# wgurecky/CORRLA_RS

Hardware: AMD Instinct MI355X
Metric: RSVD GFLOP/s on 16k x 16k f32 rank-128 (higher is better)
Workload: dtype f32

## Files before the change

### corrla_rs_amd/csrc/hip_backend.hpp

```cpp
#pragma once
#include <hip/hip_runtime.h>
#include <rccl/rccl.h>

#include <cmath>
#include <cstdio>
#include <cstdlib>
#include <cstring>
#include <limits>
#include <random>
#include <string>
#include <type_traits>
#include <vector>

#include "core_svd_plan.hpp"
#include "driver.hpp"
#include "hip_kernels.hpp"
#include "tsqr_kernels.hpp"
#include "jacobi_mc_kernels.hpp"
#include "ata_kernels.hpp"
#include "tall_kernels.hpp"
#include "mixed_kernels.hpp"
#include "grad_kernels.hpp"
#include "knn2_kernels.hpp"
#include "grad_wide_kernels.hpp"
// ... 541 lines not shown
    }
  }
  template <class T>
  void copy_values_out(const T* src_dev, int64_t n, T* dst, bool dst_is_host) {
    CORRLA_HIP(hipMemcpyAsync(dst, src_dev, sizeof(T) * n, dst_is_host ? hipMemcpyDeviceToHost : hipMemcpyDeviceToDevice,
                              stream));
    if (dst_is_host) sync();
  }
  template <class T>
  bool device_chol_fits(int64_t l) const {
    return l <= 4096 && k::chol_inv_fits((int)l, sizeof(T)) && !no_device_chol_;
  }
  template <class T>
  bool device_chol_blocked_fits(int64_t l) const {
    const int64_t n1 = round_up((l + 1) / 2, (int64_t)4);
    return l > 8 && l <= 4096 && k::chol_inv_fits((int)n1, sizeof(T)) && !no_device_chol_;
  }
  template <class T>
  void copy_block(const Skinny<T>& src, int64_t r0, int64_t c0, int64_t rows, int64_t cols, Skinny<T>& dst, int64_t dr0,
                  int64_t dc0) {
    if (rows <= 0 || cols <= 0) return;
    CORRLA_HIP(hipMemcpy2DAsync(dst.p + dc0 * dst.ld + dr0, (size_t)dst.ld * sizeof(T), src.p + c0 * src.ld + r0,
                                (size_t)src.ld * sizeof(T), (size_t)rows * sizeof(T), (size_t)cols, hipMemcpyDeviceToDevice,
                                stream));
  }
  template <class T>
  void chol_inv(const Skinny<T>& g, int64_t r, T piv_rel, Skinny<T>& m_out, void* st_dev, int slot) {
    hipLaunchKernelGGL((k::chol_inv_kernel<T>), dim3(1), dim3(k::chol_inv_threads((int)r)),
                       k::chol_inv_lds_bytes((int)r, sizeof(T)), stream, (const T*)g.p, g.ld, (int)r, piv_rel, m_out.p,
                       m_out.ld, (k::CholStatus*)st_dev + slot);
    CORRLA_HIP(hipGetLastError());
  }
  void set_run_if(const int* p) { run_if_ = p; }
  int robust_passes() const { return robust_passes_; }
  void set_robust_passes(int n) { robust_passes_ = n; }
  bool svd_more_sweeps() {
    if (jmc_extra_sweeps_ >= 24) return false;
    jmc_extra_sweeps_ += 8;
    jmc_sweeps_hint_ = 0;
    return true;
  }
  bool svd_force_v() {
    if (jmc_force_v_) return false;
    jmc_force_v_ = true;
    return true;
  }
  void svd_sweeps_used(int n) { jmc_sweeps_hint_ = std::max(jmc_sweeps_hint_ - 1, n); }
  int* alloc_flags(int n) { return (int*)alloc_zeroed(sizeof(int) * (size_t)std::max(n, 1)); }
  void* alloc_zeroed_bytes(size_t bytes) { return alloc_zeroed(bytes); }
  void read_bytes(const void* dev_p, size_t bytes, void* host) {
    CORRLA_HIP(hipMemcpyAsync(host, dev_p, bytes, hipMemcpyDeviceToHost, stream));
    sync();
  }
  template <class T>
  void poison_entry(Skinny<T>& s, int64_t i, int64_t j, int kind) {
    hipLaunchKernelGGL((k::poison_entry_kernel<T>), dim3(1), dim3(1), 0, stream, s.p + j * s.ld + i, kind);
    CORRLA_HIP(hipGetLastError());
  }
  struct ArenaMark {
    std::vector<size_t> used, zused;
  };
  ArenaMark arena_mark() const {
    ArenaMark mk;
    for (const auto& c : chunks_) mk.used.push_back(c.used);
    for (const auto& c : zchunks_) mk.zused.push_back(c.used);
    return mk;
  }
  void arena_rewind(const ArenaMark& mk) {
    sp_scratch_ = nullptr;
    sp_scratch_bytes_ = 0;
    for (size_t i = 0; i < chunks_.size(); ++i) chunks_[i].used = i < mk.used.size() ? mk.used[i] : 0;
    for (size_t i = 0; i < zchunks_.size(); ++i) {
      Chunk& c = zchunks_[i];
      const size_t keep = i < mk.zused.size() ? mk.zused[i] : 0;
      if (c.used > keep) CORRLA_HIP(hipMemsetAsync((char*)c.p + keep, 0, c.used - keep, stream));
      c.zeroed = std::max(c.zeroed, c.used);
      c.used = keep;
    }
  }
  int sharded_handshake(int local_status) {
    if (comm_size <= 1 && !(comm && env_int("CORRLA_FORCE_ALLREDUCE", 0))) return local_status;
    if (!comm) throw Error(ST_ECOMM, "communicator not initialised");
    double h[8] = {(double)local_status, (double)robust_passes_, (double)jmc_extra_sweeps_, (double)jmc_sweeps_hint_,
                   jmc_force_v_ ? 1.0 : 0.0, 0.0, 0.0, 0.0};
    double* d = (double*)alloc_bytes(sizeof(h));
    CORRLA_HIP(hipMemcpyAsync(d, h, sizeof(h), hipMemcpyHostToDevice, stream));
    CORRLA_NCCL(ncclAllReduce(d, d, 8, ncclDouble, ncclMax, comm, stream));
    ++n_collectives;
    collective_bytes += sizeof(h);
    CORRLA_HIP(hipMemcpyAsync(h, d, sizeof(h), hipMemcpyDeviceToHost, stream));
    sync();
    robust_passes_ = (int)h[1];
    jmc_extra_sweeps_ = (int)h[2];
    jmc_sweeps_hint_ = (int)h[3];
    jmc_force_v_ = h[4] != 0.0;
    return (int)h[0];
  }
  void read_flags(const int* dev_p, int n, int* host) {
    CORRLA_HIP(hipMemcpyAsync(host, dev_p, sizeof(int) * (size_t)n, hipMemcpyDeviceToHost, stream));
    sync();
  }
  template <class T>
  bool device_qr_robust_fits(int64_t l) const {
    return robust_qr_ && (device_chol_fits<T>(l) || device_chol_blocked_fits<T>(l));
  }
  bool qr_inplace_fits(int64_t l) const { return col_blocking(l).nblk == 1; }
  template <class T>
  void* alloc_inspect() { return alloc_zeroed(sizeof(k::GramInspect<T>)); }
  template <class T>
  const void* inspect_shift_ptr(const void* insp) const { return &((const k::GramInspect<T>*)insp)->shift; }
  template <class T>
  void gram_inspect(Skinny<T>& g, int64_t l, float shift_rel, int shift_mode, void* insp) {
    hipLaunchKernelGGL((k::gram_inspect_kernel<T>), dim3(1), dim3(1024), 0, stream, g.p, g.ld, (int)l, shift_rel, shift_mode,
                       (k::GramInspect<T>*)insp, run_if_);
    CORRLA_HIP(hipGetLastError());
  }
  template <class T>
  void combine_need(int* need, const void* insp, const int* na, const int* nb) {
    hipLaunchKernelGGL((k::combine_need_kernel<T>), dim3(1), dim3(1), 0, stream, need, (const k::GramInspect<T>*)insp, na, nb,
                       run_if_);
    CORRLA_HIP(hipGetLastError());
  }
  template <class T>
  void chol_inv_robust(const Skinny<T>& g, int64_t r, T piv_rel, float shift_rel, int shift_mode, float null_excess,
                       Skinny<T>& m_out, void* st_dev, int slot, int* need_next, int* null_mask,
                       const void* abs_shift = nullptr, float need_ratio = 0.f) {
    k::CholRobust rb{shift_rel, shift_mode, null_excess, need_next, null_mask, run_if_, need_ratio, abs_shift};
    hipLaunchKernelGGL((k::chol_inv_kernel<T>), dim3(1), dim3(k::chol_inv_threads((int)r)),
                       k::chol_inv_lds_bytes((int)r, sizeof(T)), stream, (const T*)g.p, g.ld, (int)r, piv_rel, m_out.p,
                       m_out.ld, (k::CholStatus*)st_dev + slot, rb);
    CORRLA_HIP(hipGetLastError());
  }
  template <class T>
  void apply_inplace(Skinny<T>& y, int64_t l, const Skinny<T>& m) {
    Skinny<T> out = y.view_cols(l);
    Skinny<T> mv = m.view_cols(l);
    mv.rows = l;
    launch_gemm<T>(true, as_rowmajor_transposed(y, l), mv, out, (const T*)nullptr);
  }
  template <class T>
  void refill_null(Skinny<T>& y, int64_t l, const int* null_mask, uint64_t seed) {
    const int bx = (int)std::min<int64_t>(64, (y.rows + 255) / 256);
    hipLaunchKernelGGL((k::refill_null_kernel<T>), dim3((unsigned)std::max(bx, 1), (unsigned)l), dim3(256), 0, stream, y.p, y.ld,
                       y.rows, (int)l, null_mask, seed, run_if_);
    CORRLA_HIP(hipGetLastError());
  }

  void read_chol_status(const void* st_dev, int n, int* fail, float* min_ratio, float* dev_i) {
    static_assert(sizeof(k::CholStatus) == 32, "driver.hpp assumes 32-byte status records");
    static_assert(k::kNeedNonFinite == kFlagNonFinite && k::kNeedNullCols == kFlagNullCols, "need_next bits: kernels vs driver");
    std::vector<k::CholStatus> h((size_t)std::max(n, 1));
    CORRLA_HIP(hipMemcpyAsync(h.data(), st_dev, sizeof(k::CholStatus) * n, hipMemcpyDeviceToHost, stream));
    sync();
    for (int i = 0; i < n; ++i) {
      fail[i] = h[i].fail;
      min_ratio[i] = h[i].min_ratio;
      dev_i[i] = h[i].dev_i;
      if (env_int("CORRLA_DEBUG", 0) >= 2)
        std::fprintf(stderr, "[corrla] chol_inv[%d]: fail %d min_ratio %.3g dev_i %.3g clk %lld wall %lld (%.0f MHz)\n", i,
                     h[i].fail, h[i].min_ratio, h[i].dev_i, h[i].clk, h[i].wall,
                     h[i].wall > 0 ? 100.0 * (double)h[i].clk / (double)h[i].wall : 0.0);
    }
  }

  template <class T>
  void inv_sqrt_series(Skinny<T>& g, int64_t r, Skinny<T>& m_out) {
    Skinny<T> e2 = alloc_skinny<T>(r, r), e3 = alloc_skinny<T>(r, r);
    if (e2.ld != g.ld || m_out.ld != g.ld) throw Error(ST_EINVAL, "internal: series operands must share a leading dimension");
    dim3 grid((unsigned)((r + 63) / 64), (unsigned)r);
    hipLaunchKernelGGL((k::series_prep_kernel<T>), grid, dim3(64), 0, stream, g.p, g.ld, (int)r);
    Big<T> eb;
    eb.p = g.p;
    eb.rows = r;
    eb.cols = r;
    eb.ld = g.ld;
    eb.cols_readable = g.ld;
    Skinny<T> gv = g.view_cols(r);
    gv.rows = r;
    gemm_nn(eb, gv, e2, (const T*)nullptr);
    gemm_nn(eb, e2, e3, (const T*)nullptr);
    memset_zero(m_out.p, (size_t)m_out.ld * m_out.cols_alloc * sizeof(T));
    hipLaunchKernelGGL((k::series_combine_kernel<T>), grid, dim3(64), 0, stream, (const T*)g.p, (const T*)e2.p,
                       (const T*)e3.p, g.ld, (int)r, m_out.p, m_out.ld);
    CORRLA_HIP(hipGetLastError());
  }

  bool hh_wy_ = env_int("CORRLA_HH_WY", 1) != 0;
  template <class T>
  size_t hh_panel_lds(int rows, int l) const {
    return hh_wy_ ? k::hh_wy_lds_bytes(rows, l, sizeof(T)) : k::hh_lds_bytes(rows, l, sizeof(T));
  }
  template <class T>
  bool householder_fits(int64_t l) const {
    return l >= 1 && l <= 4096 && hh_panel_lds<T>((int)(2 * l), (int)l) <= (size_t)160 * 1024 && 2 * l <= 64 * k::kHhMaxRowsPerLane;
  }
  template <class T>
  struct HhState {
    int64_t m = 0;
    int l = 0, nleaf = 0, levels = 0, max_rows = 0;
    std::vector<int> n_at;
    std::vector<T*> rbuf, cbuf, taub, vbuf, tbuf;
    T* r_root() const { return rbuf[levels]; }
  };
  template <class T>
  HhState<T> householder_up(Skinny<T>& y, Skinny<T>& tmp) {
    HhState<T> h;
    const int64_t m = y.rows;
    const int l = (int)y.cols;
    if (m < l) throw Error(ST_EINVAL, "householder_thin_q: fewer rows than columns");
    if (!householder_fits<T>(l)) throw Error(ST_EINVAL, "householder_thin_q: panel does not fit in LDS");
    const int64_t br = 2 * (int64_t)l;
    const int64_t nleaf64 = m <= br ? 1 : (m + br - 1) / br;
    if (nleaf64 > 0x3fffffff) throw Error(ST_EINVAL, "householder_thin_q: too many panels");
    h.m = m;
    h.l = l;
    h.nleaf = (int)nleaf64;
    h.max_rows = (int)std::min<int64_t>(m, br);
    const size_t lds = hh_panel_lds<T>(h.max_rows, l);
    h.n_at = {h.nleaf};
    while (h.n_at.back() > 1) h.n_at.push_back((h.n_at.back() + 1) / 2);
    h.levels = (int)h.n_at.size() - 1;
    const size_t ll = (size_t)l * l;
    h.rbuf.resize(h.levels + 1);
    h.cbuf.resize(h.levels + 1);
    h.taub.resize(h.levels + 1);
    h.vbuf.assign(h.levels + 1, nullptr);
    h.tbuf.assign(h.levels + 1, nullptr);
    const size_t tsz = (size_t)k::hh_wy_panels(l) * k::kWyNb * k::kWyNb;
    for (int k_ = 0; k_ <= h.levels; ++k_) {
      if (hh_wy_) h.tbuf[k_] = (T*)alloc_bytes(tsz * h.n_at[k_] * sizeof(T));
      h.rbuf[k_] = (T*)alloc_bytes(ll * h.n_at[k_] * sizeof(T));
      h.cbuf[k_] = (T*)alloc_bytes(ll * h.n_at[k_] * sizeof(T));
      h.taub[k_] = (T*)alloc_bytes((size_t)l * h.n_at[k_] * sizeof(T));
      if (k_ >= 1) h.vbuf[k_] = (T*)alloc_bytes(2 * ll * h.n_at[k_] * sizeof(T));
    }
    auto leaf = hh_wy_ ? k::hh_leaf_factor_kernel<T, true> : k::hh_leaf_factor_kernel<T, false>;
    auto tree = hh_wy_ ? k::hh_tree_factor_kernel<T, true> : k::hh_tree_factor_kernel<T, false>;
    hipLaunchKernelGGL(leaf, dim3((unsigned)h.nleaf), dim3(k::kHhThreads), lds, stream, (const T*)y.p, y.ld, m, l, h.nleaf, tmp.p,
                       tmp.ld, h.taub[0], h.rbuf[0], h.tbuf[0]);
    const size_t lds_tree = hh_panel_lds<T>(2 * l, l);
    for (int k_ = 1; k_ <= h.levels; ++k_)
      hipLaunchKernelGGL(tree, dim3((unsigned)h.n_at[k_]), dim3(k::kHhThreads), lds_tree, stream, (const T*)h.rbuf[k_ - 1],
                         h.n_at[k_ - 1], l, h.vbuf[k_], h.taub[k_], h.rbuf[k_], h.tbuf[k_]);
    CORRLA_HIP(hipGetLastError());
    return h;
  }
  template <class T>
  void householder_down(HhState<T>& h, Skinny<T>& y, Skinny<T>& tmp, const T* root_coef = nullptr) {
    const int l = h.l;
    const size_t lds = k::hh_lds_bytes(h.max_rows, l, sizeof(T));
    const size_t lds_tree = k::hh_lds_bytes(2 * l, l, sizeof(T));
    auto tree = hh_wy_ ? k::hh_tree_apply_kernel<T, true> : k::hh_tree_apply_kernel<T, false>;
    auto leaf = hh_wy_ ? k::hh_leaf_apply_kernel<T, true> : k::hh_leaf_apply_kernel<T, false>;
    for (int k_ = h.levels; k_ >= 1; --k_)
      hipLaunchKernelGGL(tree, dim3((unsigned)h.n_at[k_]), dim3(k::kHhThreads), lds_tree, stream,
                         (const T*)(k_ == h.levels ? root_coef : h.cbuf[k_]), (const T*)h.vbuf[k_], (const T*)h.taub[k_],
                         h.n_at[k_ - 1], l, h.cbuf[k_ - 1], (const T*)h.tbuf[k_]);
    hipLaunchKernelGGL(leaf, dim3((unsigned)h.nleaf), dim3(k::kHhThreads), lds, stream,
                       (const T*)(h.levels == 0 ? root_coef : h.cbuf[0]), (const T*)tmp.p, tmp.ld, (const T*)h.taub[0], h.m, l,
                       h.nleaf, y.p, y.ld, (const T*)h.tbuf[0]);
    CORRLA_HIP(hipGetLastError());
  }
  template <class T>
  void householder_thin_q(Skinny<T>& y, Skinny<T>& tmp) {
    HhState<T> h = householder_up(y, tmp);
    householder_down(h, y, tmp);
  }
  template <class T>
  int householder_max_width() const {
    int w = 1;
    while (householder_fits<T>(w + 1)) ++w;
    return w;
  }
  int rank() const { return comm_rank; }

  template <class T>
  int jmc_lanes(int64_t) const {
    return 16;
  }
  template <class T>
  bool jmc_geometry(int64_t l, int* nc_out, int* np_out, int* b_out) const {
    return corrla::jmc_geometry(l, (int)sizeof(T), jmc_lanes<T>(l), jmc_max_b_, env_int("CORRLA_JMC_LOCAL", 1),
                                env_int("CORRLA_JMC_NP", 0), nc_out, np_out, b_out);
  }
  template <class T, int NC>
  void jmc_launch_step(int lanes, int np, int b, T* w, T* v, int nblocks, int step, int sweep, T tol, T tol_early, T floor2, k::JmcCtl* ctl) {
    const size_t lds = k::jmc_lds_bytes(NC, b, sizeof(T), lanes);
    const unsigned threads = (unsigned)((b * lanes + 63) / 64 * 64);
    hipLaunchKernelGGL((k::jmc_step_kernel<T, NC, 16>), dim3((unsigned)np), dim3(threads), lds, stream, w, v, b, nblocks, step,
                       sweep, step == 0 ? 1 : 0, tol, tol_early, floor2, ctl, jmc_local_);
  }
  template <class T>
  void small_svd_mc(const Skinny<T>& c, int64_t l, int64_t k, Skinny<T>& m1, Skinny<T>& m2, T* s_dev, void* conv_status) {
    int nc = 0, np = 0, b = 0;
    if (!jmc_geometry<T>(l, &nc, &np, &b)) throw Error(ST_EINVAL, "internal: core too large for the multi-workgroup Jacobi");
    jmc_local_ = env_int("CORRLA_JMC_LOCAL", 1);
    const int lanes = jmc_lanes<T>(l);
    const int rp = k::jmc_pitch(nc, (int)sizeof(T), lanes), nblocks = 2 * np, ncols_pad = nblocks * b;
    T* wj = (T*)alloc_bytes((size_t)rp * ncols_pad * sizeof(T));
    T* vj = (T*)alloc_bytes((size_t)rp * ncols_pad * sizeof(T));
    k::JmcCtl* ctl = (k::JmcCtl*)alloc_bytes(sizeof(k::JmcCtl));
    k::CholStatus* st = conv_status ? (k::CholStatus*)conv_status : (k::CholStatus*)alloc_bytes(sizeof(k::CholStatus));
    const int force_v = (conv_status == nullptr || jmc_force_v_ || env_int("CORRLA_JMC_FORCE_V", 0)) ? 1 : 0;
    hipLaunchKernelGGL((k::jmc_init_kernel<T>), dim3(1), dim3(1024), 0, stream, (const T*)c.p, c.ld, (int)l, wj, vj, rp,
                       ncols_pad, force_v, ctl);
    const double eps = (double)std::numeric_limits<T>::epsilon();
    const T tol = (T)(std::sqrt((double)l) * eps);
    const T tol_early = env_int("CORRLA_JACOBI_STRICT", 0) ? tol : (T)std::sqrt(eps);
    const T floor2 = (T)((double)l * eps * eps);
    auto enqueue_sweeps = [&](int s0, int s1) {
      for (int sw = s0; sw < s1; ++sw)
        for (int step = 0; step < nblocks - 1; ++step) switch (nc) {
            case 1: jmc_launch_step<T, 1>(lanes, np, b, wj, vj, nblocks, step, sw, tol, tol_early, floor2, ctl); break;
            case 2: jmc_launch_step<T, 2>(lanes, np, b, wj, vj, nblocks, step, sw, tol, tol_early, floor2, ctl); break;
            case 3: jmc_launch_step<T, 3>(lanes, np, b, wj, vj, nblocks, step, sw, tol, tol_early, floor2, ctl); break;
            case 4: jmc_launch_step<T, 4>(lanes, np, b, wj, vj, nblocks, step, sw, tol, tol_early, floor2, ctl); break;
            case 5: jmc_launch_step<T, 5>(lanes, np, b, wj, vj, nblocks, step, sw, tol, tol_early, floor2, ctl); break;
            case 6: jmc_launch_step<T, 6>(lanes, np, b, wj, vj, nblocks, step, sw, tol, tol_early, floor2, ctl); break;
            case 7: jmc_launch_step<T, 7>(lanes, np, b, wj, vj, nblocks, step, sw, tol, tol_early, floor2, ctl); break;
            case 8: jmc_launch_step<T, 8>(lanes, np, b, wj, vj, nblocks, step, sw, tol, tol_early, floor2, ctl); break;
            default: jmc_launch_step<T, 9>(lanes, np, b, wj, vj, nblocks, step, sw, tol, tol_early, floor2, ctl); break;
          }
      CORRLA_HIP(hipGetLastError());
    };
    const size_t lds_fin = (size_t)(l + 2) * sizeof(T) + (size_t)(l + 2) * sizeof(int) + 64;
    auto finish = [&](int nsw) {
      hipLaunchKernelGGL((k::jmc_finish_kernel<T>), dim3(1), dim3(1024), lds_fin, stream, (const T*)wj, (const T*)vj, rp, (int)l,
                         nsw, (const k::JmcCtl*)ctl, m1.p, m1.ld, m2.p, m2.ld, s_dev, (int)k, st);
      const unsigned groups = (unsigned)(l * k);
      hipLaunchKernelGGL((k::jmc_other_factor_kernel<T>), dim3((groups * 16 + 255) / 256), dim3(256), 0, stream, (const T*)c.p,
                         c.ld, (int)l, (int)k, (const T*)m2.p, m2.ld, (const T*)s_dev, (const k::JmcCtl*)ctl, m1.p, m1.ld);
      CORRLA_HIP(hipGetLastError());
    };
    if (conv_status) {
      const int nsw_default = std::max(1, env_int("CORRLA_JMC_SWEEPS", sizeof(T) == 4 ? 10 : 13));
      const int nsw = std::min(k::kJmcMaxSweeps, (jmc_sweeps_hint_ > 0 ? std::min(nsw_default, jmc_sweeps_hint_ + 2) : nsw_default) + jmc_extra_sweeps_);
      enqueue_sweeps(0, nsw);
      finish(nsw);
      if (env_int("CORRLA_DEBUG", 0)) {
        k::JmcCtl hd;
        CORRLA_HIP(hipMemcpyAsync(&hd, ctl, sizeof(hd), hipMemcpyDeviceToHost, stream));
        sync();
        int used = 0;
        while (used < nsw && hd.rot[used] && hd.big[used]) ++used;
        std::fprintf(stderr, "[corrla] jacobi_svd (multi-workgroup, %d sweeps enqueued, %s) l=%d np=%d b=%d nc=%d sweeps run=%d rounds(wg0)=%llu "
                             "cycles/round=%.0f ns/round=%.0f (%.0f MHz)\n", nsw, hd.with_v ? "V accumulated" : "W only", (int)l, np, b, nc, std::min(used + 1, nsw),
                     hd.rounds, hd.rounds ? (double)hd.clk / hd.rounds : 0.0, hd.rounds ? 10.0 * hd.wall / hd.rounds : 0.0,
                     hd.wall ? 100.0 * hd.clk / hd.wall : 0.0);
        if (hd.steps)
          std::fprintf(stderr, "[corrla]   per step (wg0, us): load %.2f norms %.2f rounds %.2f store %.2f total %.2f over %llu steps\n",
                       0.01 * hd.t_load / hd.steps, 0.01 * hd.t_norm / hd.steps, 0.01 * hd.wall / hd.steps,
                       0.01 * hd.t_store / hd.steps, 0.01 * hd.t_total / hd.steps, hd.steps);
        if (hd.steps > 1)
          std::fprintf(stderr, "[corrla]   span first-start..last-end over all workgroups: %.2f us per step\n",
                       0.01 * hd.t_span / (hd.steps - 1));
      }
      return;
    }
    int done = 0;
    k::JmcCtl h;
    while (done < k::kJmcMaxSweeps) {
      const int s1 = std::min(k::kJmcMaxSweeps, done + 8);
      enqueue_sweeps(done, s1);
      CORRLA_HIP(hipMemcpyAsync(&h, ctl, sizeof(h), hipMemcpyDeviceToHost, stream));
      sync();
      bool conv = false;
      for (int s_ = 0; s_ < s1; ++s_) conv = conv || !(h.rot[s_] && h.big[s_]);
      done = s1;
      if (conv || h.bad) break;
    }
    if (h.bad) throw Error(ST_ENUMERIC, "non-finite core matrix in small SVD");
    finish(done);
    if (env_int("CORRLA_DEBUG", 0)) {
      int used = 0;
      while (used < done && h.rot[used] && h.big[used]) ++used;
      std::fprintf(stderr, "[corrla] jacobi_svd (multi-workgroup) l=%d np=%d b=%d sweeps=%d\n", (int)l, np, b, used + 1);
    }
  }

  template <class T>
  void small_svd(const Skinny<T>& c, int64_t l, int64_t k, Skinny<T>& m1, Skinny<T>& m2, T* s_dev, void* conv_status) {
    if (conv_status) memset_zero(conv_status, sizeof(k::CholStatus));
    CoreSvdKnobs kn;
    kn.mode = std::getenv("CORRLA_SVD");
    kn.host_svd = env_int("CORRLA_HOST_SVD", 0) != 0;
    kn.jmc_min_l = jmc_min_l_;
    kn.jmc_max_b = jmc_max_b_;
    kn.jmc_local = env_int("CORRLA_JMC_LOCAL", 1);
    kn.jmc_np = env_int("CORRLA_JMC_NP", 0);
    const CoreSvdPlan plan = core_svd_plan((int)sizeof(T), l, kn);
    switch (plan.family) {
      case CoreSvd::kMultiWg:
        small_svd_mc(c, l, k, m1, m2, s_dev, conv_status);
        return;
      case CoreSvd::kHost:
        small_svd_host(*this, c, l, k, m1, m2, s_dev);
        return;
      case CoreSvd::kBlock:
        core_finite_check<T>(c, l, conv_status);
        small_svd_block(c, l, k, m1, m2, s_dev);
        return;
      case CoreSvd::kRing:
        core_finite_check<T>(c, l, conv_status);
        small_svd_ring(c, l, k, m1, m2, s_dev, plan.ring_e);
        return;
    }
  }
  template <class T>
  void core_finite_check(const Skinny<T>& c, int64_t l, void* conv_status) {
    int* bad = conv_status ? nullptr : alloc_flags(1);
    hipLaunchKernelGGL((k::core_finite_check_kernel<T>), dim3(1), dim3(1024), 0, stream, (const T*)c.p, c.ld, (int)l,
                       (k::CholStatus*)conv_status, bad);
    CORRLA_HIP(hipGetLastError());
    if (bad) {
      int h = 0;
      read_flags(bad, 1, &h);
      if (h) throw Error(ST_ENUMERIC, "non-finite core matrix in small SVD");
    }
  }

  template <class T>
  void small_svd_block(const Skinny<T>& c, int64_t l, int64_t k, Skinny<T>& m1, Skinny<T>& m2, T* s_dev) {
    const int nb = (int)(2 * ((l + 15) / 16));
    const int cols_pad = nb * 8;
    const int rows_pad = (int)round_up(l, 16);
    const int64_t ld = rows_pad;
    T* wj = (T*)alloc_bytes((size_t)ld * cols_pad * sizeof(T));
    T* vj = (T*)alloc_bytes((size_t)ld * cols_pad * sizeof(T));
    k::JacobiCtl* ctl = (k::JacobiCtl*)alloc_bytes(sizeof(k::JacobiCtl));
    hipLaunchKernelGGL((k::jacobi_init_kernel<T>), dim3(64), dim3(256), 0, stream, (const T*)c.p, c.ld, (int)l, wj, ld, vj,
                       ld, cols_pad, rows_pad, ctl);
    const double eps = (double)std::numeric_limits<T>::epsilon();
    const float tol_early = (float)std::sqrt(eps);
    const size_t lds = (size_t)(2 * 16 * (rows_pad + 1) + 7 * 16 * 17 + 32) * sizeof(T) + 16 * sizeof(int) + 64;
    const int max_sweeps = env_int("CORRLA_JACOBI_SWEEPS", 12), inner = env_int("CORRLA_JACOBI_INNER", 1);
    for (int sw = 0; sw < max_sweeps; ++sw) {
      for (int round = 0; round < nb - 1; ++round)
        hipLaunchKernelGGL((k::jacobi_block_round_kernel<T>), dim3(nb / 2), dim3(256), lds, stream, wj, ld, vj, ld, rows_pad,
                           nb, round, inner, ctl);
      hipLaunchKernelGGL(k::jacobi_sweep_end_kernel, dim3(1), dim3(1), 0, stream, ctl, tol_early);
    }
    const size_t lds_fin = (size_t)(l + 2) * sizeof(T) + (size_t)(l + 2) * sizeof(int) + 64;
    hipLaunchKernelGGL((k::jacobi_finish_kernel<T>), dim3(1), dim3(1024), lds_fin, stream, (const T*)wj, ld, (const T*)vj,
                       ld, (int)l, m1.p, m1.ld, m2.p, m2.ld, s_dev, (int)k);
    CORRLA_HIP(hipGetLastError());
    if (env_int("CORRLA_DEBUG", 0)) {
      k::JacobiCtl h;
      CORRLA_HIP(hipMemcpyAsync(&h, ctl, sizeof(h), hipMemcpyDeviceToHost, stream));
      sync();
      std::fprintf(stderr, "[corrla] block jacobi l=%d nb=%d sweeps=%u done=%u\n", (int)l, nb, h.sweeps, h.done);
    }
  }

  template <class T>
  void small_svd_ring(const Skinny<T>& c, int64_t l, int64_t k, Skinny<T>& m1, Skinny<T>& m2, T* s_dev, int e) {
    int* info = (int*)alloc_bytes(sizeof(int) * 4);
    const double eps = (double)std::numeric_limits<T>::epsilon();
    const T tol = (T)(std::sqrt((double)l) * eps);
    const T tol_early = env_int("CORRLA_JACOBI_STRICT", 0) ? tol : (T)std::sqrt(eps);
    const size_t ring_lds = k::jacobi_ring_w_lds_bytes((int)l, 8 * e, sizeof(T));
    const int np = (int)((l + 1) / 2);
    const dim3 block((unsigned)(np * 8));
    const int max_sw = env_int("CORRLA_JACOBI_SWEEPS", 40);
    const int n2 = 2 * np;
    k::RotEntry<T>* rot = (k::RotEntry<T>*)alloc_bytes((size_t)max_sw * n2 * k::kRingProcPad * sizeof(k::RotEntry<T>));
    int* rank_g = (int*)alloc_bytes(sizeof(int) * (size_t)n2);
#define CORRLA_RING_W(EE)                                                                                             \
  hipLaunchKernelGGL((k::jacobi_ring_w_kernel<T, EE, 8>), dim3(1), block, ring_lds, stream, (const T*)c.p, c.ld, (int)l, \
                     m2.p, m2.ld, s_dev, (int)k, tol, tol_early, max_sw, rot, rank_g, info)
    constexpr int kBigE = sizeof(T) == 4 ? 20 : 18;
    switch (e) {
      case 8: CORRLA_RING_W(8); break;
      case 12: CORRLA_RING_W(12); break;
      case 16: CORRLA_RING_W(16); break;
      default: CORRLA_RING_W(kBigE); break;
    }
#undef CORRLA_RING_W
    CORRLA_HIP(hipGetLastError());
    hipLaunchKernelGGL((k::jacobi_replay_v_kernel<T>), dim3((unsigned)((l + 256 / k::kReplayLanes - 1) / (256 / k::kReplayLanes))), dim3(256), 0,
                       stream,
                       (const k::RotEntry<T>*)rot, (const int*)info, (const int*)rank_g, (int)l, (int)k, m1.p, m1.ld);
    CORRLA_HIP(hipGetLastError());
    if (env_int("CORRLA_DEBUG", 0)) {
      int h[4] = {0, 0, 0, 0};
      CORRLA_HIP(hipMemcpyAsync(h, info, sizeof(int), hipMemcpyDeviceToHost, stream));
      sync();
      std::fprintf(stderr, "[corrla] jacobi_svd (ring) l=%d sweeps=%d\n", (int)l, h[0]);
    }
  }
  template <class T>
  void copy_out(const Skinny<T>& src, int64_t ncols, T* dst, int64_t ldd, bool transpose, bool to_host) {
    const int64_t rows = src.rows;
    if (!to_host) {
      launch_copy_out(src.p, src.ld, rows, ncols, dst, ldd, transpose);
      return;
    }
    if (!transpose) {
      CORRLA_HIP(hipMemcpy2DAsync(dst, (size_t)ldd * sizeof(T), src.p, (size_t)src.ld * sizeof(T),
                                  (size_t)rows * sizeof(T), (size_t)ncols, hipMemcpyDeviceToHost, stream));
    } else {
      T* tmp = (T*)alloc_bytes((size_t)rows * ncols * sizeof(T));
      launch_copy_out(src.p, src.ld, rows, ncols, tmp, ncols, true);
      CORRLA_HIP(hipMemcpy2DAsync(dst, (size_t)ldd * sizeof(T), tmp, (size_t)ncols * sizeof(T),
                                  (size_t)ncols * sizeof(T), (size_t)rows, hipMemcpyDeviceToHost, stream));
    }
    sync();
  }
  template <class T>
  void pack_strided(const T* src, int64_t rows, int64_t cols, int64_t rs, int64_t cs, T* dst, int64_t ldd) {
    const int64_t tiles_c = (cols + 31) / 32, tiles_r = (rows + 31) / 32;
    if (tiles_c * tiles_r > 0x7fffffff) throw Error(ST_EINVAL, "problem too large for the launch grid");
    dim3 grid((unsigned)(tiles_c * tiles_r));
    hipLaunchKernelGGL((k::pack_strided_kernel<T>), grid, dim3(256), 0, stream, src, rows, cols, rs, cs, dst, ldd, tiles_c);
    CORRLA_HIP(hipGetLastError());
  }

  template <class T>
  void weighted_colsum(const Skinny<T>& x, int64_t rows, const T* w, T* v) {
    const int ncols = (int)x.cols_alloc;
    const int nblk = (int)std::max<int64_t>(1, std::min<int64_t>(64, (rows + 4095) / 4096));
    double* partial = (double*)alloc_bytes(sizeof(double) * (size_t)nblk * (size_t)ncols);
    hipLaunchKernelGGL((k::wcolsum_partial_kernel<T>), dim3((unsigned)nblk, (unsigned)ncols), dim3(256), 0, stream,
                       (const T*)x.p, x.ld, rows, w, partial, ncols);
    hipLaunchKernelGGL((k::wcolsum_final_kernel<T>), dim3((unsigned)((ncols + 63) / 64)), dim3(64), 0, stream,
                       (const double*)partial, nblk, ncols, v);
    CORRLA_HIP(hipGetLastError());
  }
  template <class T>
  void rank1_sub(Skinny<T>& out, int64_t rows, const T* u, const T* v, const T* scale) {
    dim3 grid((unsigned)((rows + 255) / 256), (unsigned)out.cols_alloc);
    check_grid(grid);
    hipLaunchKernelGGL((k::rank1_sub_kernel<T>), grid, dim3(256), 0, stream, out.p, out.ld, rows, u, v, scale);
    CORRLA_HIP(hipGetLastError());
  }

  template <class T>
  void fix_signs(Skinny<T>& v_ref, Skinny<T>& other, int64_t k) {
    hipLaunchKernelGGL((k::column_sign_apply_kernel<T>), dim3((unsigned)k), dim3(256), 0, stream, v_ref.p, v_ref.ld, v_ref.rows,
                       other.p, other.ld, other.rows);
    CORRLA_HIP(hipGetLastError());
  }
  template <class T>
  void fill_const(T* p, int64_t n, T v) {
    const int blocks = (int)std::min<int64_t>(2048, std::max<int64_t>(1, (n + 255) / 256));
    hipLaunchKernelGGL((k::fill_const_kernel<T>), dim3(blocks), dim3(256), 0, stream, p, n, v);
    CORRLA_HIP(hipGetLastError());
  }
  template <class T>
  void center_rows_cols(const T* in, int64_t rows, int64_t cols, int64_t ldi, const T* mu, bool along_cols, T* out,
                        int64_t ldo) {
    dim3 grid((unsigned)((cols + 255) / 256), (unsigned)std::min<int64_t>(rows, 4096));
    hipLaunchKernelGGL((k::center_kernel<T>), grid, dim3(256), 0, stream, in, rows, cols, ldi, mu, along_cols ? 1 : 0, out,
                       ldo);
    CORRLA_HIP(hipGetLastError());
  }

  template <class T>
  void sumsq(const Skinny<T>& y, double* out_dev) {
    const int64_t n = y.ld * y.cols_alloc;
    const int blocks = (int)std::min<int64_t>(1024, std::max<int64_t>(1, (n + 255) / 256));
    double* partial = (double*)alloc_bytes(sizeof(double) * blocks);
    hipLaunchKernelGGL((k::sumsq_partial_kernel<T>), dim3(blocks), dim3(256), 0, stream, y.p, n, partial);
    hipLaunchKernelGGL(k::sum_partials_kernel, dim3(1), dim3(64), 0, stream, partial, blocks, out_dev);
    CORRLA_HIP(hipGetLastError());
  }
  template <class T>
  void inv_norm(const Skinny<T>& y, double* ss_dev, T* inv_dev) {
    const int64_t n = y.ld * y.cols_alloc;
    const int blocks = (int)std::min<int64_t>(1024, std::max<int64_t>(1, (n + 255) / 256));
    double* partial = (double*)alloc_bytes(sizeof(double) * blocks);
    hipLaunchKernelGGL((k::sumsq_partial_kernel<T>), dim3(blocks), dim3(256), 0, stream, y.p, n, partial);
    hipLaunchKernelGGL((k::sum_partials_rsqrt_kernel<T>), dim3(1), dim3(64), 0, stream, (const double*)partial, blocks, ss_dev, inv_dev);
    CORRLA_HIP(hipGetLastError());
  }
  template <class T>
  void rsqrt_scalar(const double* ss_dev, T* out_dev) {
    hipLaunchKernelGGL((k::rsqrt_scalar_kernel<T>), dim3(1), dim3(1), 0, stream, ss_dev, out_dev);
    CORRLA_HIP(hipGetLastError());
  }
  template <class T>
  void scale_inplace(Skinny<T>& y, const T* scale_dev) {
    const int64_t n = y.ld * y.cols_alloc;
    const int blocks = (int)std::min<int64_t>(2048, std::max<int64_t>(1, (n + 255) / 256));
    hipLaunchKernelGGL((k::scale_kernel<T>), dim3(blocks), dim3(256), 0, stream, y.p, n, scale_dev);
    CORRLA_HIP(hipGetLastError());
  }
  template <class T>
  void fill_normal(T* p, int64_t rows, int64_t cols, int64_t rs, int64_t cs, uint64_t seed, int64_t row0,
                   int64_t global_cols) {
    const int64_t n = rows * cols;
    if (n <= 0) return;
    const int blocks = (int)std::min<int64_t>(8192, (n + 255) / 256);
    hipLaunchKernelGGL((k::fill_normal_kernel<T>), dim3(blocks), dim3(256), 0, stream, p, rows, cols, rs, cs, seed, row0,
                       global_cols, cs <= rs ? 1 : 0);
    CORRLA_HIP(hipGetLastError());
  }

  void set_phase_events(bool on) { phase_events_ = on; }
  void phase_end() {
    if (!phase_events_) phase_mark_impl(nullptr);
  }
  void phase_mark(double* slot) {
    if (!phase_events_ && slot != nullptr) return;
    phase_mark_impl(slot);
  }
  void phase_mark_impl(double* slot) {
    if (ev_used_ == ev_pool_.size()) {
      hipEvent_t e;
      CORRLA_HIP(hipEventCreate(&e));
      ev_pool_.push_back(e);
    }
    hipEvent_t e = ev_pool_[ev_used_++];
    CORRLA_HIP(hipEventRecord(e, stream));
    marks_.push_back({e, slot});
  }
  void phase_forget() {
    for (auto& m_ : marks_) m_.slot = nullptr;
  }
  void phase_resolve(double* total) {
    for (size_t i = 1; i < marks_.size(); ++i) {
      float ms = 0.f;
      if (hipEventElapsedTime(&ms, marks_[i - 1].ev, marks_[i].ev) != hipSuccess) {
        (void)hipGetLastError();
        continue;
      }
      if (marks_[i].slot) *marks_[i].slot += (double)ms;
    }
    if (total && marks_.size() >= 2) {
      float ms = 0.f;
      if (hipEventElapsedTime(&ms, marks_.front().ev, marks_.back().ev) == hipSuccess)
        *total = (double)ms;
      else
        (void)hipGetLastError();
    }
    marks_.clear();
  }

  void event_mark(int i) {
    CORRLA_HIP(hipEventRecord(events_[i], stream));
    events_set_[i] = true;
  }
  double event_elapsed_ms(int i, int j) {
    if (!events_set_[i] || !events_set_[j]) return 0.0;
    float ms = 0.f;
    if (hipEventElapsedTime(&ms, events_[i], events_[j]) != hipSuccess) {
      (void)hipGetLastError();
      return 0.0;
    }
    return (double)ms;
  }

  template <class F>
  double time_on_stream(int reps, F&& f) {
    hipEvent_t e0, e1;
    CORRLA_HIP(hipEventCreate(&e0));
    CORRLA_HIP(hipEventCreate(&e1));
    f();
    CORRLA_HIP(hipEventRecord(e0, stream));
    for (int i = 0; i < reps; ++i) f();
    CORRLA_HIP(hipEventRecord(e1, stream));
    CORRLA_HIP(hipEventSynchronize(e1));
    float ms = 0.f;
    CORRLA_HIP(hipEventElapsedTime(&ms, e0, e1));
    (void)hipEventDestroy(e0);
    (void)hipEventDestroy(e1);
    return (double)ms / reps;
  }

 private:
  struct Chunk {
    void* p = nullptr;
    size_t size = 0, used = 0;
    size_t zeroed = 0;
  };
  std::vector<Chunk> chunks_;
  std::vector<Chunk> zchunks_;
  void* sp_scratch_ = nullptr;
  size_t sp_scratch_bytes_ = 0;
  void* zero_page_ = nullptr;
  void* pinned_ = nullptr;
  hipEvent_t events_[3] = {nullptr, nullptr, nullptr};
  bool events_set_[3] = {false, false, false};
  struct PhaseMark {
    hipEvent_t ev;
    double* slot;
  };
  std::vector<hipEvent_t> ev_pool_;
  size_t ev_used_ = 0;
  std::vector<PhaseMark> marks_;
  static constexpr size_t kPinnedBytes = (size_t)8 << 20;
  int gemm_debug_flags_ = 0;
  GemmKnobs gemm_knobs_;
  uint64_t entropy_ = 0, calls_ = 0, calls_sharded_ = 0;
// ... 206 lines not shown
```

### corrla_rs_amd/csrc/jacobi_mc_kernels.hpp

```cpp
#pragma once
#include "core_svd_plan.hpp"
#include "hip_kernels.hpp"

namespace corrla {
namespace k {

constexpr int kJmcMaxSweeps = 40;
constexpr float kJmcFastCond = 16.f;
constexpr float kJmcVerifyCond = 64.f;
struct JmcCtl {
  unsigned rot[kJmcMaxSweeps + 1];
  unsigned big[kJmcMaxSweeps + 1];
  int sexp;
  int bad;
  int with_v;
  unsigned long long clk, wall;
  unsigned long long rounds;
  unsigned long long t_load, t_norm, t_store, t_total, steps;
  unsigned long long t_max_total;
  unsigned long long t_first, t_last;
  unsigned long long t_span;
};

template <class T>
struct JmcVec;
template <>
struct JmcVec<float> {
  typedef float v2 __attribute__((ext_vector_type(2)));
};
template <>
struct JmcVec<double> {
  typedef double v2 __attribute__((ext_vector_type(2)));
};

template <int LANES>
__device__ __forceinline__ float jmc_sum(float x) {
  return group_sum<LANES>(x);
}
template <int LANES>
__device__ __forceinline__ double jmc_sum(double x) {
  static_assert(LANES == 16, "f64 processors are 16 lanes wide");
  auto dpp = [](double v, auto ctrl) {
    int lo = __double2loint(v), hi = __double2hiint(v);
    lo = __builtin_amdgcn_update_dpp(0, lo, decltype(ctrl)::value, 0xf, 0xf, true);
    hi = __builtin_amdgcn_update_dpp(0, hi, decltype(ctrl)::value, 0xf, 0xf, true);
    return __hiloint2double(hi, lo);
  };
  x += dpp(x, std::integral_constant<int, 0xB1>{});
  x += dpp(x, std::integral_constant<int, 0x4E>{});
  x += dpp(x, std::integral_constant<int, 0x141>{});
  x += dpp(x, std::integral_constant<int, 0x140>{});
  return x;
}


template <class T>
__global__ __launch_bounds__(1024) void jmc_init_kernel(const T* __restrict__ c, int64_t ldc, int l, T* w, T* v, int rp,
                                                        int ncols_pad, int force_v, JmcCtl* ctl) {
  __shared__ float red[16];
  __shared__ int sbad;
  const int tid = threadIdx.x;
  if (tid == 0) sbad = 0;
  float mx = 0.f;
  int bad = 0;
  for (int idx0 = tid; idx0 < l * l; idx0 += 4 * 1024) {
    T xb[4];
#pragma unroll
    for (int u = 0; u < 4; ++u) {
      const int idx = min(idx0 + u * 1024, l * l - 1);
      const int j = idx / l, i = idx - j * l;
      xb[u] = c[(int64_t)j * ldc + i];
    }
#pragma unroll
    for (int u = 0; u < 4; ++u)
      if (idx0 + u * 1024 < l * l) {
        const float x = (float)fabs(xb[u]);
        if (!(x < 3.0e38f)) bad = 1;
        mx = fmaxf(mx, x);
      }
  }
  for (int off = 32; off > 0; off >>= 1) mx = fmaxf(mx, __shfl_xor(mx, off, 64));
  if ((tid & 63) == 0) red[tid >> 6] = mx;
  __syncthreads();
  if (bad) sbad = 1;
  mx = 0.f;
  for (int i = 0; i < 16; ++i) mx = fmaxf(mx, red[i]);
  __syncthreads();
  int sexp = 0;
  if (mx > 0.f && !sbad) {
    (void)frexpf(mx, &sexp);
    sexp = 1 - sexp;
  }
  const int total = rp * ncols_pad;
  for (int idx0 = tid; idx0 < total; idx0 += 4 * 1024) {
    T xb[4];
#pragma unroll
    for (int u = 0; u < 4; ++u) {
      const int idx = min(idx0 + u * 1024, total - 1);
      const int j = idx / rp, i = idx - j * rp;
      xb[u] = c[(int64_t)min(j, l - 1) * ldc + min(i, l - 1)];
    }
#pragma unroll
    for (int u = 0; u < 4; ++u) {
      const int idx = idx0 + u * 1024;
      if (idx < total) {
        const int j = idx / rp, i = idx - j * rp;
        const bool in = i < l && j < l;
        w[idx] = in ? (T)ldexp((double)xb[u], sexp) : (T)0;
        v[idx] = (in && i == j) ? (T)1 : (T)0;
      }
    }
  }
  for (int i = tid; i <= kJmcMaxSweeps; i += 1024) {
    ctl->rot[i] = 0;
    ctl->big[i] = 0;
  }
  float dmin = 3.0e38f, dmax = 0.f;
  for (int i = tid; i < l; i += 1024) {
    const float d = (float)fabs(c[(int64_t)i * ldc + i]);
    dmin = fminf(dmin, d);
    dmax = fmaxf(dmax, d);
  }
  for (int off = 32; off > 0; off >>= 1) {
    dmin = fminf(dmin, __shfl_xor(dmin, off, 64));
    dmax = fmaxf(dmax, __shfl_xor(dmax, off, 64));
  }
  __shared__ float rmin[16], rmax[16];
  if ((tid & 63) == 0) {
    rmin[tid >> 6] = dmin;
    rmax[tid >> 6] = dmax;
  }
  __syncthreads();
  if (tid == 0) {
    for (int i = 0; i < 16; ++i) {
      dmin = fminf(dmin, rmin[i]);
      dmax = fmaxf(dmax, rmax[i]);
    }
    ctl->with_v = (force_v || !(dmin * kJmcFastCond >= dmax) || !(dmax > 0.f)) ? 1 : 0;
    ctl->sexp = sexp;
    ctl->bad = sbad;
    ctl->clk = 0;
    ctl->wall = 0;
    ctl->rounds = 0;
    ctl->t_load = ctl->t_norm = ctl->t_store = ctl->t_total = ctl->steps = 0;
    ctl->t_max_total = ctl->t_span = 0;
    ctl->t_first = ~0ull;
    ctl->t_last = 0;
  }
}

__device__ __forceinline__ bool jmc_rotation_flat(float a, float b, float g, float tol, float tol_early, float floor2,
                                                  float& cs, float& sn, float& t, bool& big) {
  const float g2 = g * g, ab = a * b;
  const float zeta = (b - a) * 0.5f * __builtin_amdgcn_rcpf(g);
  const float den = fabsf(zeta) + __builtin_amdgcn_sqrtf(1.f + zeta * zeta);
  const float t_ = copysignf(__builtin_amdgcn_rcpf(den), zeta);
  const float c_ = __builtin_amdgcn_rsqf(1.f + t_ * t_);
  const float s_ = c_ * t_;
  const bool ok = (a > floor2) && (b > floor2) && (g2 > (tol * tol) * ab) && (fabsf(s_) <= 1.f) && (c_ <= 1.f);
  big = ok && (g2 > (tol_early * tol_early) * ab);
  cs = ok ? c_ : 1.f;
  sn = ok ? s_ : 0.f;
  t = ok ? t_ : 0.f;
  return ok;
}
__device__ __forceinline__ bool jmc_rotation_flat(double a, double b, double g, double tol, double tol_early, double floor2,
                                                  double& cs, double& sn, double& t, bool& big) {
  const double g2 = g * g, ab = a * b;
  const double zeta = (b - a) * 0.5 * jr_rcp(g);
  const double w = 1.0 + zeta * zeta;
  const double den = fabs(zeta) + w * jr_rsq(w);
  const double t_ = copysign(jr_rcp(den), zeta);
  const double c_ = jr_rsq(1.0 + t_ * t_);
  const double s_ = c_ * t_;
  const bool ok = (a > floor2) && (b > floor2) && (g2 > (tol * tol) * ab) && (fabs(s_) <= 1.0) && (c_ <= 1.0);
  big = ok && (g2 > (tol_early * tol_early) * ab);
  cs = ok ? c_ : 1.0;
  sn = ok ? s_ : 0.0;
  t = ok ? t_ : 0.0;
  return ok;
}

template <class T, int NC, int LANES>
__global__ __launch_bounds__(512) void jmc_step_kernel(T* w, T* v, int b, int nblocks, int step, int sweep, int within,
                                                        T tol, T tol_early, T floor2, JmcCtl* ctl, int local) {
  typedef typename JmcVec<T>::v2 v2;
  constexpr int PITCH = jmc_pitch(NC, (int)sizeof(T), LANES);
  const int sp = sweep > 0 ? sweep - 1 : 0;
  const unsigned rot_prev = ctl->rot[sp], big_prev = ctl->big[sp];
  const int bad_in = ctl->bad, with_v_in = ctl->with_v;
  if (sweep > 0 && !(rot_prev && big_prev)) return;
  if (bad_in) return;
  if (threadIdx.x == 0 && blockIdx.x == 0 && ctl->t_last != 0) {
    ctl->t_span += ctl->t_last - ctl->t_first;
    ctl->t_first = ~0ull;
    ctl->t_last = 0;
  }
  extern __shared__ __attribute__((aligned(16))) char smem[];
  T* wl = (T*)smem;
  T* vl = wl + (size_t)2 * b * PITCH;
  T* nrm = vl + (size_t)2 * b * PITCH;
  int* flag = (int*)(nrm + 2 * b);
  const int tid = threadIdx.x, nthr = blockDim.x;
  const int proc = tid / LANES, g = tid % LANES;
  const bool act = proc < b;
  int bp, bq;
  tournament_pair(nblocks, step, blockIdx.x, bp, bq);
  if (tid < 2) flag[tid] = 0;
  const bool with_v = with_v_in != 0;
  const long long ts0 = wall_clock64();
  const int lane = tid & 63;
  const int wave = __builtin_amdgcn_readfirstlane(tid >> 6), nwaves = (nthr + 63) >> 6;
  const int seg_bytes = b * PITCH * (int)sizeof(T);
  {
    const char* src[4] = {(const char*)(w + (int64_t)bp * b * PITCH), (const char*)(w + (int64_t)bq * b * PITCH),
                          (const char*)(v + (int64_t)bp * b * PITCH), (const char*)(v + (int64_t)bq * b * PITCH)};
    char* dst[4] = {(char*)wl, (char*)(wl + (size_t)b * PITCH), (char*)vl, (char*)(vl + (size_t)b * PITCH)};
    const int nch = (seg_bytes + 1023) >> 10;
    const int nseg = with_v ? 4 : 2;
#pragma unroll
    for (int sgi = 0; sgi < 4; ++sgi)
      if (sgi < nseg)
      for (int c = wave; c < nch; c += nwaves) {
        const int off = c * 1024 + lane * 16;
        if (off < seg_bytes) glds16(src[sgi] + off, dst[sgi] + c * 1024);
      }
    asm volatile("s_waitcnt vmcnt(0)" ::: "memory");
  }
  __syncthreads();
  const long long ts1 = wall_clock64();
  const int lane_off = g * 2;
  if (act) {
#pragma unroll
    for (int h = 0; h < 2; ++h) {
      const int s = proc + h * b;
      const T* col = wl + (size_t)s * PITCH + lane_off;
      T a0 = 0, a1 = 0;
#pragma unroll
      for (int c = 0; c < NC; ++c) {
        const v2 x = *(const v2*)(col + c * 2 * LANES);
        a0 += x[0] * x[0];
        a1 += x[1] * x[1];
      }
      const T a = jmc_sum<LANES>(a0 + a1);
      if (g == 0) nrm[s] = a;
    }
  }
  __syncthreads();
  int my_rot = 0, my_big = 0;
  auto round = [&](int sx, int sy) {
    T* cx = wl + (size_t)sx * PITCH + lane_off;
    T* cy = wl + (size_t)sy * PITCH + lane_off;
    T* ux = vl + (size_t)sx * PITCH + lane_off;
    T* uy = vl + (size_t)sy * PITCH + lane_off;
    v2 x[NC], y[NC], vx[NC], vy[NC];
#pragma unroll
    for (int c = 0; c < NC; ++c) {
      x[c] = *(const v2*)(cx + c * 2 * LANES);
      y[c] = *(const v2*)(cy + c * 2 * LANES);
    }
    if (with_v) {
#pragma unroll
      for (int c = 0; c < NC; ++c) {
        vx[c] = *(const v2*)(ux + c * 2 * LANES);
        vy[c] = *(const v2*)(uy + c * 2 * LANES);
      }
    }
    T na = nrm[sx], nb = nrm[sy];
    v2 acc = x[0] * y[0];
#pragma unroll
    for (int c = 1; c < NC; ++c) acc += x[c] * y[c];
    const T gg = jmc_sum<LANES>(acc[0] + acc[1]);
    T cs, sn, rel, t;
    if (na > floor2 && nb > floor2 && jacobi_rotation(na, nb, gg, tol, cs, sn, rel, t)) {
      my_rot = 1;
      if (rel > tol_early) my_big = 1;
#pragma unroll
      for (int c = 0; c < NC; ++c) {
        *(v2*)(cx + c * 2 * LANES) = cs * x[c] - sn * y[c];
        *(v2*)(cy + c * 2 * LANES) = sn * x[c] + cs * y[c];
      }
      if (with_v) {
#pragma unroll
        for (int c = 0; c < NC; ++c) {
          *(v2*)(ux + c * 2 * LANES) = cs * vx[c] - sn * vy[c];
          *(v2*)(uy + c * 2 * LANES) = sn * vx[c] + cs * vy[c];
        }
      }
      if (g == 0) {
        nrm[sx] = na - t * gg;
        nrm[sy] = nb + t * gg;
      }
    }
  };
  const long long clk0 = clock64(), wall0 = wall_clock64();
  const long long ts2 = wall0;
  auto inner4 = [&](auto wv, v2 (&x)[NC], v2 (&vx)[NC], T& na, int sb0) {
    constexpr bool WV = decltype(wv)::value;
    const int pi = proc & 3;
    constexpr bool DB = !(WV && sizeof(T) == 8 && NC > 4);
    constexpr int NB = DB ? 2 : 1;
    v2 y[NB][NC];
    T nb[NB];
    auto fetch = [&](int r, int buf) {
      const int sy = sb0 + ((pi + r) & 3);
      const T* cy = wl + (size_t)sy * PITCH + lane_off;
      nb[buf] = nrm[sy];
#pragma unroll
      for (int c = 0; c < NC; ++c) y[buf][c] = *(const v2*)(cy + c * 2 * LANES);
    };
    fetch(0, 0);
#pragma unroll
    for (int r = 0; r < 4; ++r) {
      const int cur = DB ? (r & 1) : 0;
      const int sy = sb0 + ((pi + r) & 3);
      T* cy = wl + (size_t)sy * PITCH + lane_off;
      T* uy = vl + (size_t)sy * PITCH + lane_off;
      v2 acc = x[0] * y[cur][0], acc2 = {0, 0};
      if (NC > 1) acc2 = x[1] * y[cur][1];
#pragma unroll
      for (int c = 2; c < NC; c += 2) {
        acc += x[c] * y[cur][c];
        if (c + 1 < NC) acc2 += x[c + 1] * y[cur][c + 1];
      }
      acc += acc2;
      const T gg = jmc_sum<LANES>(acc[0] + acc[1]);
      T cs, sn, t;
      bool big;
      const bool rot = jmc_rotation_flat(na, nb[cur], gg, tol, tol_early, floor2, cs, sn, t, big);
      my_rot |= rot ? 1 : 0;
      my_big |= big ? 1 : 0;
      const bool any = __builtin_amdgcn_ballot_w64(rot) != 0;
      if (any) {
#pragma unroll
        for (int c = 0; c < NC; ++c) *(v2*)(cy + c * 2 * LANES) = sn * x[c] + cs * y[cur][c];
        if (g == 0) nrm[sy] = nb[cur] + t * gg;
      }
      asm volatile("" ::: "memory");
      if (DB && r < 3) fetch(r + 1, cur ^ 1);
      if (any) {
      if (WV) {
        v2 vy[NC];
#pragma unroll
        for (int c = 0; c < NC; ++c) vy[c] = *(const v2*)(uy + c * 2 * LANES);
#pragma unroll
        for (int c = 0; c < NC; ++c) {
          *(v2*)(uy + c * 2 * LANES) = sn * vx[c] + cs * vy[c];
          vx[c] = cs * vx[c] - sn * vy[c];
        }
      }
#pragma unroll
      for (int c = 0; c < NC; ++c) x[c] = cs * x[c] - sn * y[cur][c];
      na -= t * gg;
      }
      if (!DB && r < 3) fetch(r + 1, 0);
    }
  };
  auto load_col = [&](auto wv, int slot, v2 (&x)[NC], v2 (&vx)[NC], T& na) {
    const T* cx = wl + (size_t)slot * PITCH + lane_off;
    const T* ux = vl + (size_t)slot * PITCH + lane_off;
#pragma unroll
    for (int c = 0; c < NC; ++c) x[c] = *(const v2*)(cx + c * 2 * LANES);
    if (decltype(wv)::value) {
#pragma unroll
      for (int c = 0; c < NC; ++c) vx[c] = *(const v2*)(ux + c * 2 * LANES);
    }
    na = nrm[slot];
  };
  auto store_col = [&](auto wv, int slot, const v2 (&x)[NC], const v2 (&vx)[NC], T na) {
    T* cx = wl + (size_t)slot * PITCH + lane_off;
    T* ux = vl + (size_t)slot * PITCH + lane_off;
#pragma unroll
    for (int c = 0; c < NC; ++c) *(v2*)(cx + c * 2 * LANES) = x[c];
    if (decltype(wv)::value) {
#pragma unroll
      for (int c = 0; c < NC; ++c) *(v2*)(ux + c * 2 * LANES) = vx[c];
    }
    if (g == 0) nrm[slot] = na;
  };
  auto run_local = [&](auto wv) {
    const int nsb = b >> 2;
    const int pi = proc & 3;
    v2 x[NC], vx[NC];
    T na = 0;
    {
      load_col(wv, proc, x, vx, na);
      for (int s = 0; s < nsb; ++s) {
        int m = wave + s;
        if (m >= nsb) m -= nsb;
        inner4(wv, x, vx, na, b + 4 * m);
        __syncthreads();
      }
      store_col(wv, proc, x, vx, na);
      __syncthreads();
    }
    if (within) {
      const int n_even = nsb + (nsb & 1), halfn = n_even >> 1;
      const int real = (nsb & 1) ? halfn - 1 : halfn;
      const int side = real > 0 ? wave / real : 2, jj = real > 0 ? wave - side * real : 0;
      for (int t_ = 0; t_ < n_even - 1; ++t_) {
        if (side < 2) {
          int pa = -1, pb = -1, cnt = 0;
          for (int j = 0; j < halfn; ++j) {
            int p_, q_;
            tournament_pair(n_even, t_, j, p_, q_);
            if (q_ < nsb) {
              if (cnt == jj) {
                pa = p_;
                pb = q_;
              }
              ++cnt;
            }
          }
          if (pa >= 0) {
            const int sa = side * b + 4 * pa + pi;
            load_col(wv, sa, x, vx, na);
            inner4(wv, x, vx, na, side * b + 4 * pb);
            store_col(wv, sa, x, vx, na);
          }
        }
        __syncthreads();
      }
      {
        const int base = (pi >> 1) * b + 4 * wave;
#pragma unroll
        for (int t_ = 0; t_ < 3; ++t_) {
          int p_, q_;
          tournament_pair(4, t_, pi & 1, p_, q_);
          round(base + p_, base + q_);
          asm volatile("" ::: "memory");
        }
      }
      __syncthreads();
    }
  };
  if (local && LANES == 16 && (b & 3) == 0) {
    if (with_v)
      run_local(std::true_type{});
    else
      run_local(std::false_type{});
// ... 232 lines not shown
```

Before: 92040.

## Parallelize Jacobi init across workgroups and trim spare sweeps and memset

The Jacobi init kernel now runs on up to 16 workgroups. Each workgroup redundantly computes the max-abs scale, then writes a grid-strided slice of the padded W/V buffers. The diagonal min/max is folded into the first scan instead of a separate pass, and the scan unroll grows from 4 to 8. The spare sweep margin over the hint drops from 2 to 1, and the status memset is skipped on the multi-workgroup path, which removes Jacobi sweep launches and one memset at some risk to convergence margin.

Result: no change. 92500 (median of 2 runs) (+0.5%).

```diff
diff --git a/corrla_rs_amd/csrc/hip_backend.hpp b/corrla_rs_amd/csrc/hip_backend.hpp
--- a/corrla_rs_amd/csrc/hip_backend.hpp
+++ b/corrla_rs_amd/csrc/hip_backend.hpp
@@ -867,8 +867,9 @@
     k::JmcCtl* ctl = (k::JmcCtl*)alloc_bytes(sizeof(k::JmcCtl));
     k::CholStatus* st = conv_status ? (k::CholStatus*)conv_status : (k::CholStatus*)alloc_bytes(sizeof(k::CholStatus));
     const int force_v = (conv_status == nullptr || jmc_force_v_ || env_int("CORRLA_JMC_FORCE_V", 0)) ? 1 : 0;
-    hipLaunchKernelGGL((k::jmc_init_kernel<T>), dim3(1), dim3(1024), 0, stream, (const T*)c.p, c.ld, (int)l, wj, vj, rp,
-                       ncols_pad, force_v, ctl);
+    const unsigned init_wgs = (unsigned)std::min<int64_t>(16, ((int64_t)rp * ncols_pad + 4095) / 4096);
+    hipLaunchKernelGGL((k::jmc_init_kernel<T>), dim3(std::max(init_wgs, 1u)), dim3(1024), 0, stream, (const T*)c.p, c.ld, (int)l,
+                       wj, vj, rp, ncols_pad, force_v, ctl);
     const double eps = (double)std::numeric_limits<T>::epsilon();
     const T tol = (T)(std::sqrt((double)l) * eps);
     const T tol_early = env_int("CORRLA_JACOBI_STRICT", 0) ? tol : (T)std::sqrt(eps);
@@ -899,7 +900,7 @@
     };
     if (conv_status) {
       const int nsw_default = std::max(1, env_int("CORRLA_JMC_SWEEPS", sizeof(T) == 4 ? 10 : 13));
-      const int nsw = std::min(k::kJmcMaxSweeps, (jmc_sweeps_hint_ > 0 ? std::min(nsw_default, jmc_sweeps_hint_ + 2) : nsw_default) + jmc_extra_sweeps_);
+      const int nsw = std::min(k::kJmcMaxSweeps, (jmc_sweeps_hint_ > 0 ? std::min(nsw_default, jmc_sweeps_hint_ + k::kJmcSpareSweeps) : nsw_default) + jmc_extra_sweeps_);
       enqueue_sweeps(0, nsw);
       finish(nsw);
       if (env_int("CORRLA_DEBUG", 0)) {
@@ -945,7 +946,6 @@
 
   template <class T>
   void small_svd(const Skinny<T>& c, int64_t l, int64_t k, Skinny<T>& m1, Skinny<T>& m2, T* s_dev, void* conv_status) {
-    if (conv_status) memset_zero(conv_status, sizeof(k::CholStatus));
     CoreSvdKnobs kn;
     kn.mode = std::getenv("CORRLA_SVD");
     kn.host_svd = env_int("CORRLA_HOST_SVD", 0) != 0;
@@ -954,6 +954,7 @@
     kn.jmc_local = env_int("CORRLA_JMC_LOCAL", 1);
     kn.jmc_np = env_int("CORRLA_JMC_NP", 0);
     const CoreSvdPlan plan = core_svd_plan((int)sizeof(T), l, kn);
+    if (conv_status && plan.family != CoreSvd::kMultiWg) memset_zero(conv_status, sizeof(k::CholStatus));
     switch (plan.family) {
       case CoreSvd::kMultiWg:
         small_svd_mc(c, l, k, m1, m2, s_dev, conv_status);
diff --git a/corrla_rs_amd/csrc/jacobi_mc_kernels.hpp b/corrla_rs_amd/csrc/jacobi_mc_kernels.hpp
--- a/corrla_rs_amd/csrc/jacobi_mc_kernels.hpp
+++ b/corrla_rs_amd/csrc/jacobi_mc_kernels.hpp
@@ -6,6 +6,7 @@
 namespace k {
 
 constexpr int kJmcMaxSweeps = 40;
+constexpr int kJmcSpareSweeps = 1;
 constexpr float kJmcFastCond = 16.f;
 constexpr float kJmcVerifyCond = 64.f;
 struct JmcCtl {
@@ -57,34 +58,54 @@
 template <class T>
 __global__ __launch_bounds__(1024) void jmc_init_kernel(const T* __restrict__ c, int64_t ldc, int l, T* w, T* v, int rp,
                                                         int ncols_pad, int force_v, JmcCtl* ctl) {
-  __shared__ float red[16];
+  __shared__ float red[16], rmin[16], rmax[16];
   __shared__ int sbad;
   const int tid = threadIdx.x;
   if (tid == 0) sbad = 0;
   float mx = 0.f;
   int bad = 0;
-  for (int idx0 = tid; idx0 < l * l; idx0 += 4 * 1024) {
-    T xb[4];
-#pragma unroll
-    for (int u = 0; u < 4; ++u) {
+  float dmin = 3.0e38f, dmax = 0.f;
+  for (int idx0 = tid; idx0 < l * l; idx0 += 8 * 1024) {
+    T xb[8];
+#pragma unroll
+    for (int u = 0; u < 8; ++u) {
       const int idx = min(idx0 + u * 1024, l * l - 1);
       const int j = idx / l, i = idx - j * l;
       xb[u] = c[(int64_t)j * ldc + i];
     }
 #pragma unroll
-    for (int u = 0; u < 4; ++u)
-      if (idx0 + u * 1024 < l * l) {
+    for (int u = 0; u < 8; ++u) {
+      const int idx = idx0 + u * 1024;
+      if (idx < l * l) {
         const float x = (float)fabs(xb[u]);
         if (!(x < 3.0e38f)) bad = 1;
         mx = fmaxf(mx, x);
-      }
-  }
-  for (int off = 32; off > 0; off >>= 1) mx = fmaxf(mx, __shfl_xor(mx, off, 64));
-  if ((tid & 63) == 0) red[tid >> 6] = mx;
+        const int j = idx / l, i = idx - j * l;
+        if (i == j) {
+          dmin = fminf(dmin, x);
+          dmax = fmaxf(dmax, x);
+        }
+      }
+    }
+  }
+  for (int off = 32; off > 0; off >>= 1) {
+    mx = fmaxf(mx, __shfl_xor(mx, off, 64));
+    dmin = fminf(dmin, __shfl_xor(dmin, off, 64));
+    dmax = fmaxf(dmax, __shfl_xor(dmax, off, 64));
+  }
+  if ((tid & 63) == 0) {
+    red[tid >> 6] = mx;
+    rmin[tid >> 6] = dmin;
+    rmax[tid >> 6] = dmax;
+  }
   __syncthreads();
   if (bad) sbad = 1;
   mx = 0.f;
-  for (int i = 0; i < 16; ++i) mx = fmaxf(mx, red[i]);
+  for (int i = 0; i < 16; ++i) {
+    mx = fmaxf(mx, red[i]);
+    dmin = fminf(dmin, rmin[i]);
+    dmax = fmaxf(dmax, rmax[i]);
+  }
   __syncthreads();
   int sexp = 0;
   if (mx > 0.f && !sbad) {
@@ -92,17 +113,18 @@
     sexp = 1 - sexp;
   }
   const int total = rp * ncols_pad;
-  for (int idx0 = tid; idx0 < total; idx0 += 4 * 1024) {
+  const int gthreads = (int)gridDim.x * 1024;
+  for (int idx0 = (int)blockIdx.x * 1024 + tid; idx0 < total; idx0 += 4 * gthreads) {
     T xb[4];
 #pragma unroll
     for (int u = 0; u < 4; ++u) {
-      const int idx = min(idx0 + u * 1024, total - 1);
+      const int idx = min(idx0 + u * gthreads, total - 1);
       const int j = idx / rp, i = idx - j * rp;
       xb[u] = c[(int64_t)min(j, l - 1) * ldc + min(i, l - 1)];
     }
 #pragma unroll
     for (int u = 0; u < 4; ++u) {
-      const int idx = idx0 + u * 1024;
+      const int idx = idx0 + u * gthreads;
       if (idx < total) {
         const int j = idx / rp, i = idx - j * rp;
         const bool in = i < l && j < l;
@@ -111,31 +133,12 @@
       }
     }
   }
+  if (blockIdx.x != 0) return;
   for (int i = tid; i <= kJmcMaxSweeps; i += 1024) {
     ctl->rot[i] = 0;
     ctl->big[i] = 0;
   }
-  float dmin = 3.0e38f, dmax = 0.f;
-  for (int i = tid; i < l; i += 1024) {
-    const float d = (float)fabs(c[(int64_t)i * ldc + i]);
-    dmin = fminf(dmin, d);
-    dmax = fmaxf(dmax, d);
-  }
-  for (int off = 32; off > 0; off >>= 1) {
-    dmin = fminf(dmin, __shfl_xor(dmin, off, 64));
-    dmax = fmaxf(dmax, __shfl_xor(dmax, off, 64));
-  }
-  __shared__ float rmin[16], rmax[16];
-  if ((tid & 63) == 0) {
-    rmin[tid >> 6] = dmin;
-    rmax[tid >> 6] = dmax;
-  }
-  __syncthreads();
   if (tid == 0) {
-    for (int i = 0; i < 16; ++i) {
-      dmin = fminf(dmin, rmin[i]);
-      dmax = fmaxf(dmax, rmax[i]);
-    }
     ctl->with_v = (force_v || !(dmin * kJmcFastCond >= dmax) || !(dmax > 0.f)) ? 1 : 0;
     ctl->sexp = sexp;
     ctl->bad = sbad;
```
